# ISLA-UH/quantum-inferno

Measured on AMD Instinct MI355X. Metric: TFR Mpoints/sec (CWT+STX+entropy), higher is better.
Workload: dtype f32; 1 GPU; BASELINE configs[1]: 1 channel(s) per GPU x 2^20 samples @ 1000 Hz, order N=3, CWT+STX+entropy, 48 bands; channels_per_gpu=1, n=1048576, bands=48, engine=auto, world_size=1, backend=none, gather_message_bytes_per_rank=0

## Files before the change

### quantum_inferno_amd/csrc/qi_block.hip

```cpp
#include "qi_common.hpp"
#include "qi_device.hpp"
#include "qi_native.hpp"
#include "qi_fft_reg.hpp"
#include "qi_zoom_gather.hpp"

namespace qi {
namespace native {

namespace {

constexpr int kBlkThreads = 256;
#ifndef QI_BLK_WAVES
#define QI_BLK_WAVES 3
#endif
#ifndef QI_BLK_LONG_WAVES
#define QI_BLK_LONG_WAVES 2
#endif
#ifdef QI_NATIVE_DEBUG
#define QI_BDBG(bit) (a.debug & (bit))
#else
#define QI_BDBG(bit) false
#endif
#ifdef QI_NATIVE_STAMPS
#define QI_BSTAMP(k)                                               \
// ... 451 lines not shown
    }
    QI_BSTAMP(4);
  }
#ifdef QI_NATIVE_STAMPS
  if (a.stamps && tid == 0) {
    unsigned long long* o = a.stamps + ((int64_t)blockIdx.z * gridDim.x + blockIdx.x) * 8;
    for (int k = 0; k < 5; ++k) o[k] = st_acc[k];
    o[5] = (unsigned long long)band_count;
  }
#endif

  T tot = T(0);
  char* __restrict__ time_row = reinterpret_cast<char*>(
      a.time_part ? a.time_part + ((int64_t)ch * a.chunk_total + a.chunk_base + plane) * n : nullptr);
#pragma unroll
  for (int i = 0; i < NOUT; i += 2) {
    tot += col_p[i] + col_p[i + 1];
    const uint32_t tt = tb_pair + 256u * (uint32_t)i;
    if (time_row && tt < (uint32_t)n) store_real_pair(time_row, tt, col_p[i], col_p[i + 1]);
  }
  const double r0 = wave_max((double)mx), r1 = wave_sum((double)tot), r2 = wave_sum(plogp);
  __syncthreads();
  if (pending >= 0 && tid == 0) {
    double r = 0.0;
    for (int q = 0; q < NW; ++q) r += s_red[par ^ 1][q];
    a.part_band[((int64_t)ch * a.panel_bands + pending) * a.nblk + blk] = r;
  }
  if (a.part_stat) {
    double* fin = reinterpret_cast<double*>(buf);
    if (lane == 0) {
      fin[wv] = r0;
      fin[NW + wv] = r1;
// ... 732 lines not shown
  cplx<T> w;
  {
    float s, c;
    sincospif((float)col * (2.0f / 4096.0f), &s, &c);
    w = mk<T>((T)c, (T)s);
  }
  fft4096<T, 1>(v, buf, tw256, w, tid, col);
#pragma unroll
  for (int c = 0; c < 16; ++c) plane[256 * c] = v[brev(c, 4)];
}
template <typename T, bool STX, int NF>
__device__ __forceinline__ void zoom_coarse_plane_gather(const ZoomArgs<T>& a, const uint32_t plane_i,
                                                         cplx<T>* __restrict__ buf, cplx<T>* __restrict__ tw256) {
  const int tid = threadIdx.x, lane = tid & (kWave - 1);
  const int col = (tid & ~(kWave - 1)) + (lane < 32 ? 2 * lane : 2 * (lane - 32) + 1);
  const BandDesc bd = load_uniform(a.bands + *as_const(a.plane_band + plane_i));
  const uint32_t tau1 = plane_i - (uint32_t)bd.edge;
  const int64_t ch = blockIdx.z;
  const cplx<T>* __restrict__ X = a.X + ch * (a.Lf << a.x_shift);
  cplx<T> v[16];
#ifdef QI_NATIVE_DEBUG
  if (a.debug & 256) {
#pragma unroll
    for (int b = 0; b < 16; ++b) v[b] = mk<T>((T)(col + b), (T)tau1);
  } else
#endif
  zoom_gather16<T, STX, NF>(a, bd, tau1, col, X, v);
  {
    float s, c;
    sincospif((float)tid * (2.0f / 256.0f), &s, &c);
    tw256[tid] = mk<T>((T)c, (T)s);
// ... 428 lines not shown
```

### quantum_inferno_amd/csrc/qi_host.hpp

```cpp
#pragma once
#include <algorithm>
#include <cmath>
#include <cstring>
#include <map>
#include <mutex>
#include <new>
#include <tuple>
#include <vector>

#include <cstdlib>

#include "qi_common.hpp"
#include "qi_native.hpp"

namespace qi {

struct DeviceGuard {
  int prev = -1;
  bool ok = true;
  explicit DeviceGuard(int dev) {
    if (hipGetDevice(&prev) != hipSuccess) prev = -1;
    if (prev != dev) ok = hipSetDevice(dev) == hipSuccess;
  }
  ~DeviceGuard() {
// ... 183 lines not shown
  Profiler prof;
  struct NativeGroup {
    int32_t first = 0, count = 0;
    int32_t gen_first = 0, ngen = 0;
  };
  struct NativeTable {
    bool ready = false;
    int64_t Lf = 0;
    int32_t nbands = 0, ngen = 0, imd_slots = 0;
    native::BandDesc* d_bands = nullptr;
    int32_t* d_gen_list = nullptr;
    std::vector<NativeGroup> groups;
    void* Hc = nullptr;
    void* Hfull = nullptr;
    native::BandDesc* d_zoom = nullptr;
    int32_t* d_zoom_plane_band = nullptr;
    std::vector<std::pair<int32_t, int32_t>> h_zoom;
    std::vector<int32_t> h_rows;
    int32_t nzoom = 0, zoom_count[native::kZoomClasses] = {0, 0, 0, 0, 0, 0, 0};
    int64_t zoom_planes = 0;
    int zoom_max_level = 0;
    native::BandDesc* d_z64 = nullptr;
    int32_t nz64 = 0, z64_first[native::kZ64Levels] = {}, z64_count[native::kZ64Levels] = {};
    int32_t zf_first[native::kZ64FineClasses] = {}, zf_count[native::kZ64FineClasses] = {};
    double2* d_z64_lane_ph = nullptr;
    double2* d_z64_wave_ph = nullptr;
    void release() {
      if (d_z64) (void)hipFree(d_z64);
      if (d_z64_lane_ph) (void)hipFree(d_z64_lane_ph);
      if (d_z64_wave_ph) (void)hipFree(d_z64_wave_ph);
      if (d_zoom) (void)hipFree(d_zoom);
      if (d_zoom_plane_band) (void)hipFree(d_zoom_plane_band);
      if (d_bands) (void)hipFree(d_bands);
      if (d_gen_list) (void)hipFree(d_gen_list);
      if (Hc) (void)hipFree(Hc);
      if (Hfull) (void)hipFree(Hfull);
      *this = NativeTable();
    }
  } nat[4];
  struct BlockTable {
    bool ready = false;
    int demod = 0;
    void* bank = nullptr;
    int32_t rows = 0;
    struct ItemList {
      void* d_bands = nullptr;
      void* d_demod_pow = nullptr;
      void* d_gauss_w = nullptr;
      std::vector<std::pair<int32_t, int32_t>> h_bands;
      native::BlockItem* d_items = nullptr;
      int32_t nitems = 0, nplanes = 0;
      int32_t nlong = 0;
      int32_t nedge_items = 0;
      bool edge_merged = false;
      std::vector<native::BlockItem> h_items;
    } var[2];
    int64_t max_blocks = 0;
    void release() {
      if (bank) (void)hipFree(bank);
      for (auto& v : var) {
        if (v.d_bands) (void)hipFree(v.d_bands);
        if (v.d_demod_pow) (void)hipFree(v.d_demod_pow);
        if (v.d_gauss_w) (void)hipFree(v.d_gauss_w);
        if (v.d_items) (void)hipFree(v.d_items);
      }
      *this = BlockTable();
// ... 121 lines not shown
```

### quantum_inferno_amd/csrc/qi_native.hip

```cpp
#include <utility>

#include "qi_common.hpp"
#include "qi_device.hpp"
#include "qi_native.hpp"
#include "qi_fft_reg.hpp"
#include "qi_finalize.hpp"

namespace qi {
namespace native {

namespace {

template <typename T, int G_ = 16>
struct Cfg {
  static constexpr int NR = 1024, G = G_, TH = 64 * G_;
  static constexpr int SR = NR + 1;
  static constexpr int SA = 16 * G + 1;
  static constexpr int BUF = (G * SR > 64 * SA) ? G * SR : 64 * SA;
  static constexpr int TW1 = (kMaxPrunedTerms + 1) * G;
  static constexpr int TW2 = 64;
  static constexpr size_t LDS_BYTES = ((size_t)BUF + NR + TW2 + TW1) * sizeof(cplx<T>) + 256;
};

#ifdef QI_NATIVE_DEBUG
// ... 476 lines not shown
      double m = 0.0, s1 = 0.0, s2 = 0.0;
      for (int w = 0; w < C::TH / kWave; ++w) {
        m = s_fin[0][w] > m ? s_fin[0][w] : m;
        s1 += s_fin[1][w];
        s2 += s_fin[2][w];
      }
      double* o = a.part_stat + ((int64_t)ch * a.stat_stride + (int64_t)(a.chunk_base + blockIdx.y) * a.stat_nblk + grp) * 3;
      o[0] = m;
      o[1] = s1;
      o[2] = s2;
    }
  }
}

template <typename T, int VEC>
__device__ __forceinline__ void time_reduce_block(const T* __restrict__ part, T* __restrict__ out, int64_t n, int nchunk,
                                                  const T* __restrict__ edge_time, int64_t wmax, int64_t bx, int64_t gx,
                                                  int64_t c) {
  struct alignas(sizeof(T) * VEC) Pack {
    T v[VEC];
  };
  for (int64_t t = (bx * blockDim.x + threadIdx.x) * VEC; t < n; t += gx * blockDim.x * VEC) {
    if (t + VEC <= n) {
      Pack s = *reinterpret_cast<const Pack*>(part + (c * nchunk) * n + t);
      for (int q = 1; q < nchunk; ++q) {
        const Pack x = *reinterpret_cast<const Pack*>(part + (c * nchunk + q) * n + t);
#pragma unroll
        for (int i = 0; i < VEC; ++i) s.v[i] += x.v[i];
      }
      if (edge_time) {
#pragma unroll
        for (int i = 0; i < VEC; ++i) {
          if (t + i < wmax) s.v[i] += edge_time[(c * 2 + 0) * wmax + t + i];
          if (t + i >= n - wmax) s.v[i] += edge_time[(c * 2 + 1) * wmax + (n - 1 - t - i)];
        }
      }
      *reinterpret_cast<Pack*>(out + c * n + t) = s;
    } else {
      for (int64_t u = t; u < n; ++u) {
        T s = T(0);
        for (int q = 0; q < nchunk; ++q) s += part[(c * nchunk + q) * n + u];
        if (edge_time) {
          if (u < wmax) s += edge_time[(c * 2 + 0) * wmax + u];
          if (u >= n - wmax) s += edge_time[(c * 2 + 1) * wmax + (n - 1 - u)];
        }
        out[c * n + u] = s;
      }
    }
  }
}
template <typename T, int VEC>
__global__ void __launch_bounds__(256) k_time_reduce(const T* __restrict__ part, T* __restrict__ out, int64_t n, int nchunk,
                                                     const T* __restrict__ edge_time, int64_t wmax) {
  time_reduce_block<T, VEC>(part, out, n, nchunk, edge_time, wmax, blockIdx.x, gridDim.x, blockIdx.y);
}

struct TailFin {
  const double* part_band;
  const double* part_stat;
  double* power_band;
  double* stats;
  int64_t B, nblk, nstat;
  const int32_t* band_slots;
};
template <typename T, int VEC>
__global__ void __launch_bounds__(256) k_tail(const T* __restrict__ part, T* __restrict__ out, int64_t n, int nchunk,
                                              const T* __restrict__ edge_time, int64_t wmax, TailFin f, int nfin) {
  __shared__ double s[3][256 / kWave];
  if ((int)blockIdx.x < nfin) {
    finalize_block(f.part_band, f.part_stat, f.power_band, f.stats, f.B, f.nblk, f.nstat, f.band_slots, blockIdx.x,
                   blockIdx.y, s);
    return;
  }
  time_reduce_block<T, VEC>(part, out, n, nchunk, edge_time, wmax, (int64_t)blockIdx.x - nfin, (int64_t)gridDim.x - nfin,
                            blockIdx.y);
}

template <typename T>
__global__ void k_even_bins(const cplx<T>* __restrict__ x2, cplx<T>* __restrict__ x1, int64_t n) {
  const int64_t k = (int64_t)blockIdx.x * blockDim.x + threadIdx.x, c = blockIdx.y;
  if (k < n) x1[c * n + k] = x2[c * 2 * n + 2 * k];
}

template <typename T>
__global__ void __launch_bounds__(256) k_edge_fix(EdgeArgs<T> a) {
  const int lane = threadIdx.x & (kWave - 1), wv = threadIdx.x / kWave;
  const int64_t e = blockIdx.y, c = blockIdx.z;
  const EdgeBand eb = a.bands[e];
  const int64_t o = (int64_t)blockIdx.x * (256 / kWave) + wv;
// ... 300 lines not shown
    return QI_ERR_UNSUPPORTED;
  }
  return launch_pass2_cfg<double, Cfg<double, 8>>(a, kind, nchunk, n_channels, st);
}

template <>
int launch_pass2<float>(const RowArgs<float>& a, int kind, int rows_per_group, int nchunk, int64_t n_channels,
                        hipStream_t st) {
  if (rows_per_group == 16) return launch_pass2_cfg<float, Cfg<float, 16>>(a, kind, nchunk, n_channels, st);
  if (rows_per_group == 8) return launch_pass2_cfg<float, Cfg<float, 8>>(a, kind, nchunk, n_channels, st);
  set_error("pass 2 supports 8 or 16 rows per workgroup, got %d", rows_per_group);
  return QI_ERR_UNSUPPORTED;
}

template <typename T>
int launch_time_reduce(const T* part, T* out, int64_t C, int64_t n, int nchunk, const T* edge_time, int64_t wmax,
                       hipStream_t st) {
  const bool aligned = n % 4 == 0 && reinterpret_cast<uintptr_t>(out) % (4 * sizeof(T)) == 0 &&
                       reinterpret_cast<uintptr_t>(part) % (4 * sizeof(T)) == 0;
  if (aligned) {
    dim3 g((unsigned)(ceil_div(n, 1024) > 4096 ? 4096 : ceil_div(n, 1024)), (unsigned)C);
    k_time_reduce<T, 4><<<g, 256, 0, st>>>(part, out, n, nchunk, edge_time, wmax);
  } else {
    dim3 g((unsigned)(ceil_div(n, 256) > 4096 ? 4096 : ceil_div(n, 256)), (unsigned)C);
    k_time_reduce<T, 1><<<g, 256, 0, st>>>(part, out, n, nchunk, edge_time, wmax);
  }
  QI_LAUNCH_CHECK();
  return QI_OK;
}
template <typename T>
struct TailPack {
  const T* part;
  T* out;
  int64_t n;
  int nchunk, nfin;
  TailFin f;
};
template <typename T, int VEC>
__global__ void __launch_bounds__(256) k_tail2(TailPack<T> p0, TailPack<T> p1) {
  __shared__ double s[3][256 / kWave];
  const TailPack<T>& p = blockIdx.z == 0 ? p0 : p1;
  if ((int)blockIdx.x < p.nfin) {
    finalize_block(p.f.part_band, p.f.part_stat, p.f.power_band, p.f.stats, p.f.B, p.f.nblk, p.f.nstat, p.f.band_slots,
                   blockIdx.x, blockIdx.y, s);
    return;
  }
  time_reduce_block<T, VEC>(p.part, p.out, p.n, p.nchunk, nullptr, 0, (int64_t)blockIdx.x - p.nfin,
                            (int64_t)gridDim.x - p.nfin, blockIdx.y);
}

template <typename T>
int launch_tail(const TailCall<T>& t, hipStream_t st) {
  const bool aligned = t.n % 4 == 0 && reinterpret_cast<uintptr_t>(t.out_time) % (4 * sizeof(T)) == 0 &&
                       reinterpret_cast<uintptr_t>(t.time_part) % (4 * sizeof(T)) == 0;
  if (!aligned) {
    if (int rc = launch_time_reduce<T>(t.time_part, t.out_time, t.ct, t.n, t.chunk_total, t.edge_time, t.wmax, st)) return rc;
    return launch_finalize(t.part_band, t.part_stat, t.power_band, t.stats, t.ct, t.B, t.nbk, t.stat_slots, st, t.band_slots);
  }
  const TailFin f{t.part_band, t.part_stat, t.power_band, t.stats, t.B, t.nbk, t.stat_slots, t.band_slots};
  const int nfin = (int)t.B + 1;
  const int64_t gt = ceil_div(t.n, 1024) > 4096 ? 4096 : ceil_div(t.n, 1024);
  dim3 g((unsigned)(gt + nfin), (unsigned)t.ct);
  k_tail<T, 4><<<g, 256, 0, st>>>(t.time_part, t.out_time, t.n, t.chunk_total, t.edge_time, t.wmax, f, nfin);
  QI_LAUNCH_CHECK();
  return QI_OK;
}

template <typename T>
int launch_tail2(const TailCall<T>& t0, const TailCall<T>& t1, hipStream_t st) {
  const int64_t n = t1.n;
  const bool aligned = n % 4 == 0 && reinterpret_cast<uintptr_t>(t0.out_time) % 16 == 0 &&
                       reinterpret_cast<uintptr_t>(t0.time_part) % 16 == 0 && reinterpret_cast<uintptr_t>(t1.out_time) % 16 == 0 &&
                       reinterpret_cast<uintptr_t>(t1.time_part) % 16 == 0;
  if (!aligned) {
    if (int rc = launch_tail<T>(t0, st)) return rc;
    return launch_tail<T>(t1, st);
  }
  TailPack<T> p0{t0.time_part, t0.out_time, n, t0.chunk_total, (int)t0.B + 1,
                 TailFin{t0.part_band, t0.part_stat, t0.power_band, t0.stats, t0.B, t0.nbk, t0.stat_slots, t0.band_slots}};
  TailPack<T> p1{t1.time_part, t1.out_time, n, t1.chunk_total, (int)t1.B + 1,
                 TailFin{t1.part_band, t1.part_stat, t1.power_band, t1.stats, t1.B, t1.nbk, t1.stat_slots, t1.band_slots}};
  const int64_t gt = ceil_div(n, 1024) > 4096 ? 4096 : ceil_div(n, 1024);
  const int nfin = p0.nfin > p1.nfin ? p0.nfin : p1.nfin;
  dim3 g((unsigned)(gt + nfin), (unsigned)t1.ct, 2);
  k_tail2<T, 4><<<g, 256, 0, st>>>(p0, p1);
  QI_LAUNCH_CHECK();
  return QI_OK;
}
template int launch_tail2<float>(const TailCall<float>&, const TailCall<float>&, hipStream_t);
template int launch_tail<float>(const TailCall<float>&, hipStream_t);
template int launch_tail<double>(const TailCall<double>&, hipStream_t);
template int launch_time_reduce<float>(const float*, float*, int64_t, int64_t, int, const float*, int64_t, hipStream_t);
template int launch_time_reduce<double>(const double*, double*, int64_t, int64_t, int, const double*, int64_t,
                                        hipStream_t);

template <typename T>
int launch_even_bins(const cplx<T>* x2, cplx<T>* x1, int64_t C, int64_t n, hipStream_t st) {
  dim3 g((unsigned)ceil_div(n, 256), (unsigned)C);
  k_even_bins<T><<<g, 256, 0, st>>>(x2, x1, n);
  QI_LAUNCH_CHECK();
  return QI_OK;
}
template int launch_even_bins<float>(const float2*, float2*, int64_t, int64_t, hipStream_t);
template int launch_even_bins<double>(const double2*, double2*, int64_t, int64_t, hipStream_t);

template <typename T>
int launch_edge(const EdgeArgs<T>& a, int64_t C, T* edge_time, double* part_band, int64_t nblk, int64_t band_slot,
                double* part_stat, int64_t stat_slot, hipStream_t st) {
// ... 35 lines not shown
```

### quantum_inferno_amd/csrc/qi_native.hpp

```cpp
#pragma once
#include "qi_common.hpp"

namespace qi {
namespace native {

constexpr int kN2 = 1024;
constexpr int kMaxPrunedTerms = 16;

struct BandDesc {
  int32_t mode;
  int32_t k_lo;
  int32_t k_len;
  int32_t gen_slot;
  int32_t out_band;
  int32_t bank_row;
  int32_t edge;
  int32_t edge_slot;
  int32_t add_row;
  int32_t pad_;
  int64_t src_off;
  int64_t shift;
  double coef;
};

// ... 103 lines not shown
  const BlockItem* items;
  const BlockBandT<T>* bands;
  const cplx<T>* bank;
  const T* gauss_w;
  const cplx<T>* demod_pow;
  const cplx<T>* demod_t1;
  const cplx<T>* demod_t2;
  const T* sig;
  cplx<T>* coef;
  T* bits;
  T* time_part;
  double* part_band;
  double* part_stat;
  int64_t nblk, stat_stride, stat_base;
  int32_t chunk_base, chunk_total;
  T power_scale, eps;
  float two_over_n;
  int32_t debug;
  unsigned long long* stamps;
};
int block_valid(int wq);
template <typename T>
int launch_block(const BlockArgs<T>& a, int demod, int64_t n_channels, hipStream_t st, hipStream_t side = nullptr,
                 hipEvent_t fork = nullptr, hipEvent_t join = nullptr);
template <typename T>
int launch_block_dual(const BlockArgs<T>& a0, const BlockArgs<T>& a2, const DualItem* items, int32_t nitems, int32_t nlong,
                      int32_t n_edge, int64_t n_channels, hipStream_t st);
int launch_block_taps_gabor(double2* g, int w, const double* d_par, int nb_total, const int32_t* d_ids, int count,
                            hipStream_t st);
int launch_block_taps_stx(double2* g, int w, const double2* om, int64_t n, int64_t idx, hipStream_t st);
// ... 7 lines not shown
constexpr int kZoomLevels = 5;
constexpr int kZoomClasses = 7;
constexpr int zoom_grid(int cls) { return cls < kZoomLevels ? cls : 0; }
constexpr int zoom_ntap(int cls) { return cls < kZoomLevels ? 10 : (cls == 5 ? 6 : 4); }
constexpr int zoom_design_oversampling(int cls) { return cls < kZoomLevels ? 4 : (cls == 5 ? 8 : 32); }
constexpr int zoom_span(int cls) { return 1 << zoom_grid(cls); }
constexpr int zoom_taps(int cls) { return zoom_ntap(cls) + zoom_span(cls) - 1; }
constexpr int zoom_steps(int cls) { return zoom_grid(cls) <= 2 ? 16 : (64 >> zoom_grid(cls)); }
constexpr int kZoomOversample = 4;
template <typename T>
struct ZoomArgs {
  int64_t n, Lf;
  int64_t planes;
  int32_t nbands, panel_bands;
  const BandDesc* bands;
  const int32_t* plane_band;
  int32_t lvl_first[kZoomClasses], lvl_count[kZoomClasses], lvl_chunk0[kZoomClasses], lvl_nchunk[kZoomClasses];
  int64_t lvl_stat_base[kZoomClasses];
  const float* lvl_weights[kZoomClasses];
  const cplx<T>* X;
  int32_t x_shift;
  const cplx<T>* Hc;
  cplx<T>* split_part;
  int32_t split_rows;
  int32_t debug;
  cplx<T>* coarse;
  int32_t stx;
  int32_t lane_off;
  int64_t tau_off;
  T inv_len;
  float two_over_len;
// ... 73 lines not shown
  int32_t cls;
  int32_t nrow;
  int32_t lvl_bands;
  int32_t lvl_index0;
  const double* w;
  const cplx<double>* lane_ph;
  const cplx<double>* wave_ph;
  int32_t debug;
};
int launch_z64_fine(const Z64FineArgs& a, int64_t n_channels, hipStream_t st);
void z64_fine_weights(int cls, double* w );

void zoom_weights(int level, int lane_off, float* w );

template <typename T>
int launch_time_reduce(const T* part, T* out, int64_t C, int64_t n, int nchunk, const T* edge_time, int64_t wmax,
                       hipStream_t st);
template <typename T>
struct TailCall {
  const T* time_part = nullptr;
  T* out_time = nullptr;
  int64_t ct = 0, n = 0;
  int chunk_total = 0;
  const T* edge_time = nullptr;
  int64_t wmax = 0;
  const double* part_band = nullptr;
  const double* part_stat = nullptr;
  double* power_band = nullptr;
  double* stats = nullptr;
  int64_t B = 0, nbk = 0, stat_slots = 0;
  const int32_t* band_slots = nullptr;
};
template <typename T>
int launch_tail(const TailCall<T>& t, hipStream_t st);
template <typename T>
int launch_tail2(const TailCall<T>& t0, const TailCall<T>& t1, hipStream_t st);
template <typename T>
int launch_even_bins(const cplx<T>* x2, cplx<T>* x1, int64_t C, int64_t n, hipStream_t st);
// ... 11 lines not shown
```

### quantum_inferno_amd/csrc/qi_plan_build.hip

```cpp
#include <algorithm>

#include "qi_host.hpp"

using namespace qi;

namespace qi {
namespace host {

bool native_len_ok(int64_t Lf) { return Lf == (1ll << 20) || Lf == (1ll << 21); }

bool native_wanted(const qi_plan* p, int kind) {
  if (p->d.engine == QI_ENGINE_HIPFFT) return false;
  const int64_t Lf = kind == 0 ? p->L : p->n;
  if (p->d.dtype == QI_F64 && !p->native_f64) return false;
  if (is_pow2(p->n) && native_len_ok(Lf)) return true;
  return kind != 1 && is_pow2(p->n) && p->n >= ((int64_t)1 << p->native_min_log2n) && Lf <= (1ll << 26);
}

bool z64_table(const qi_plan* p, int table) { return p->d.dtype == QI_F64 && p->native_z64 && table != 3; }
int64_t narrow_limit(const qi_plan* p, int table, int64_t Lf) {
  return z64_table(p, table) ? std::max<int64_t>(p->native_kmax, Lf >> (9 - p->native_z64_levels)) : p->native_kmax;
}

int batch_from(const qi_plan* p) {
// ... 38 lines not shown
      const int g = kZoomListOrder[gi];
      const int grid = native::zoom_grid(g);
      for (auto d : by_level[g]) {
        d.edge_slot = grid;
        d.edge = (int32_t)t.zoom_planes;
        t.zoom_planes += ((Lf / native::kZoomD) << grid) / native::kBlk;
        if (grid > t.zoom_max_level) t.zoom_max_level = grid;
        zoom.push_back(d);
        t.h_zoom.push_back({d.out_band, g});
      }
    }
    if (!zoom.empty()) {
      QI_HIP(hipMalloc((void**)&t.d_zoom, zoom.size() * sizeof(native::BandDesc)));
      QI_HIP(hipMemcpy(t.d_zoom, zoom.data(), zoom.size() * sizeof(native::BandDesc), hipMemcpyHostToDevice));
      t.nzoom = (int32_t)zoom.size();
      std::vector<int32_t> owner((size_t)t.zoom_planes);
      for (size_t j = 0; j < zoom.size(); ++j) {
        const int64_t planes = ((Lf / native::kZoomD) << zoom[j].edge_slot) / native::kBlk;
        for (int64_t q = 0; q < planes; ++q) owner[(size_t)(zoom[j].edge + q)] = (int32_t)j;
      }
      QI_HIP(hipMalloc((void**)&t.d_zoom_plane_band, owner.size() * sizeof(int32_t)));
      QI_HIP(hipMemcpy(t.d_zoom_plane_band, owner.data(), owner.size() * sizeof(int32_t), hipMemcpyHostToDevice));
      for (int g = 0; g < native::kZoomClasses; ++g)
        for (int e = 0; e < 1; ++e) {
          const bool needed = t.zoom_count[g] > 0 || (g == 0 && t.zoom_count[5] + t.zoom_count[6] > 0);
          if (p->d_zoom_w[g][e] || !needed) continue;
          std::vector<float> w((size_t)64 * native::zoom_taps(g));
          native::zoom_weights(g, e, w.data());
          QI_HIP(hipMalloc((void**)&p->d_zoom_w[g][e], w.size() * sizeof(float)));
          QI_HIP(hipMemcpy(p->d_zoom_w[g][e], w.data(), w.size() * sizeof(float), hipMemcpyHostToDevice));
        }
    }
    bands.swap(rest);
  }
  if (z64_table(p, kind)) {
    std::vector<native::BandDesc> rest;
    std::vector<std::vector<native::BandDesc>> lvl(native::kZ64Levels);
// ... 333 lines not shown
        {
          const int64_t m1 = picks[r].shift % p->n;
          b.rot1[0] = (T)std::cos(-2.0 * M_PI * (double)m1 / (double)p->n);
          b.rot1[1] = (T)std::sin(-2.0 * M_PI * (double)m1 / (double)p->n);
        }
        list.push_back(b);
      }
      group_first[g] = first;
      group_count[g] = (int32_t)list.size() - first;
      if (group_count[g] == 0) continue;
      const int64_t nblocks = ceil_div(p->n, native::block_valid(wqs[g]));
      if (nblocks > bt.max_blocks) bt.max_blocks = nblocks;
      for (int32_t q = first; q < (int32_t)list.size(); ++q) il.h_bands.push_back({list[q].out_band, (int32_t)nblocks});
    }
    std::vector<native::BlockItem> items;
    for (int g = 0; g < NG; ++g) {
      const int32_t first = group_first[g], count = group_count[g];
      if (count == 0) continue;
      const int per_wg = v == 0 ? p->native_blk_bands : p->native_blk_bands_batch;
      const int32_t nchunk = (int32_t)ceil_div(count, per_wg);
      const int64_t nblocks = ceil_div(p->n, native::block_valid(wqs[g]));
      if (tune_env("QI_NATIVE_VERBOSE"))
        fprintf(stderr, "[qi plan] block table %d cut %d, reach <= %d%s: %d bands (%d analytic, %d narrow, %d half) in %d workgroups x %lld blocks\n", kind, v,
                g == 3 ? 1024 : 256 * (wqs[g] & 15), g == 3 ? " (8192-sample blocks)" : "", count,
                (int)std::count_if(list.begin() + first, list.begin() + first + count, [](const native::BlockBandT<T>& b) { return b.analytic != 0; }),
                (int)std::count_if(list.begin() + first, list.begin() + first + count, [](const native::BlockBandT<T>& b) { return b.narrow == 1; }),
                (int)std::count_if(list.begin() + first, list.begin() + first + count, [](const native::BlockBandT<T>& b) { return b.narrow == 2; }),
                nchunk, (long long)nblocks);
      for (int32_t c = 0; c < nchunk; ++c) {
        const int32_t lo = first + (int32_t)((int64_t)count * c / nchunk);
        const int32_t hi = first + (int32_t)((int64_t)count * (c + 1) / nchunk);
        for (int64_t b = 0; b < nblocks; ++b) {
          native::BlockItem it;
          it.wq = wqs[g];
          it.block = (int32_t)b;
          it.band_first = lo;
          it.band_count = hi - lo;
          it.plane = il.nplanes;
          it.stat_slot = 0;
          items.push_back(it);
        }
        il.nplanes += 1;
      }
    }
    std::stable_sort(items.begin(), items.end(), [](const native::BlockItem& x, const native::BlockItem& y) {
      const bool lx = x.wq == native::kBlkLongWq, ly = y.wq == native::kBlkLongWq;
      return lx != ly ? lx : x.band_count > y.band_count;
    });
    for (size_t i = 0; i < items.size(); ++i) items[i].stat_slot = (int32_t)i;
    il.nitems = (int32_t)items.size();
    il.nlong = (int32_t)std::count_if(items.begin(), items.end(), [](const native::BlockItem& x) { return x.wq == native::kBlkLongWq; });
    if (kind == 0 && p->nsplit > 0) {
      const int wq = (int)(p->native_split_e / 512);
      il.edge_merged = (v == 1 && p->native_edge_merge != 0) || F64;
      if (il.edge_merged) {
// ... 484 lines not shown
```

### quantum_inferno_amd/csrc/qi_run.hip

```cpp
#include "qi_host.hpp"

using namespace qi;

namespace qi {
namespace host {



struct Tile {
  int64_t Ct, Bt, ntb, nblk;
  size_t off_x, off_y, off_pb, off_ps;
};

template <typename T>
int plan_tiles(const qi_plan* p, int64_t C, int64_t B, int64_t L, Tile* t) {
  const size_t row = (size_t)L * sizeof(cplx<T>);
  const int64_t nblk = ceil_div(p->n, kEpiSpan);
  const size_t part = align_up((size_t)B * nblk * 8) + align_up((size_t)B * nblk * 24);
  const size_t per_chan_full = row * (size_t)(B + 1) + part + 2048;
  int64_t Ct, Bt;
  if (per_chan_full <= p->ws_bytes) {
    Bt = B;
    Ct = (int64_t)(p->ws_bytes / per_chan_full);
    if (Ct > C) Ct = C;
// ... 533 lines not shown
  v.fill_panel(e);
  e.edge_z = s.edge_z;
  e.edge_p = s.edge_p;
  return native::launch_edge<T>(e, ct, v.out_time ? s.edge_time : nullptr, v.part_band, v.nbk, v.nbk - 1, v.part_stat,
                                v.stat_slots - p->nedge, st);
}

template <typename T>
native::TailCall<T> tail_call(const TileOut<T>& v, int64_t ct, const int32_t* band_slots) {
  native::TailCall<T> t;
  t.time_part = v.time_part;
  t.out_time = v.out_time;
  t.ct = ct;
  t.n = v.n;
  t.chunk_total = v.chunk_total;
  t.part_band = v.part_band;
  t.part_stat = v.part_stat;
  t.power_band = v.power_band;
  t.stats = v.stats;
  t.B = v.B;
  t.nbk = v.nbk;
  t.stat_slots = v.stat_slots;
  t.band_slots = band_slots;
  return t;
}

template <typename T>
int launch_reductions(const native::TailCall<T>& t, bool time_via_part, bool one_launch, hipStream_t st) {
  const bool sums = t.part_band || t.part_stat;
  if (time_via_part && sums && one_launch) return native::launch_tail<T>(t, st);
  if (time_via_part)
    QI_TRY(native::launch_time_reduce<T>(t.time_part, t.out_time, t.ct, t.n, t.chunk_total, t.edge_time, t.wmax, st));
  if (sums)
    QI_TRY(launch_finalize(t.part_band, t.part_stat, t.power_band, t.stats, t.ct, t.B, t.nbk, t.stat_slots, st, t.band_slots));
  return QI_OK;
}


struct ZoomRows {
  int count[native::kZoomClasses] = {}, nchunk[native::kZoomClasses] = {};
  int64_t stat_base[native::kZoomClasses] = {}, groups[native::kZoomClasses] = {};
  int planes = 0;
  int64_t stats = 0, slots = 0;
};

ZoomRows plan_zoom_rows(const qi_plan* p, int kind, int64_t C, bool joint) {
  constexpr int NL = native::kZoomClasses;
// ... 70 lines not shown
  return QI_OK;
}

native::ZoomArgs<float> zoom_args(const qi_plan* p, int kind, const ZoomRows& r, const TileOut<float>& v, const Scratch<float>& s,
                                  bool x_shift, int32_t nsplit, int64_t stat_base, int chunk_base) {
  using T = float;
  const auto& zt = p->nat[kind];
  const int64_t n = v.n;
  native::ZoomArgs<T> z{};
  z.n = n;
  z.Lf = zt.Lf;
  z.planes = zt.zoom_planes;
  z.nbands = zt.nzoom;
  z.panel_bands = (int32_t)v.B;
  z.bands = zt.d_zoom;
  z.plane_band = zt.d_zoom_plane_band;
  z.X = s.X;
  z.x_shift = x_shift ? 1 : 0;
  z.Hc = static_cast<const cplx<T>*>(zt.Hc);
  z.coarse = s.zoom;
  z.stx = kind == 2 ? 1 : 0;
  z.lane_off = kind == 0 ? 1 : 0;
  z.tau_off = kind == 2 ? 0 : n / 2 / native::kZoomD;
  z.inv_len = (T)(1.0 / (double)zt.Lf);
  z.two_over_len = (float)(2.0 / (double)zt.Lf);
  v.fill(z);
  z.chunk_base = chunk_base;
  z.split_part = s.zadd;
  z.split_rows = nsplit;
  z.debug = p->native_debug;
  int chunk0 = 0;
// ... 108 lines not shown
    blk_stats = il.nitems + il.nedge_items;
    blk_slots = bt.max_blocks;
  }
  const auto& zt = p->nat[kind];
  const bool zoom = zt.nzoom > 0;
  const ZoomRows zr = plan_zoom_rows(p, kind, C, defer || (finish && (finish->active || probe)));
  const int chunk_z0 = chunk_total;
  chunk_total += zr.planes;
  int64_t nbk = tp.nblk_max + (shorts ? 1 : 0);
  if (blk_slots > nbk) nbk = blk_slots;
  if (zr.slots > nbk) nbk = zr.slots;
  const int64_t p2_stats = (int64_t)chunk_p2 * tp.nblk_max;
  const int64_t stat_slots = p2_stats + blk_stats + zr.stats + (shorts ? p->nedge : 0);
  const bool sums = out->power_band || out->stats;
  const bool time_via_part = out->power_time && (chunk_total > 1 || shorts);
  if (!shorts) QI_TRY(upload_band_slots(p, kind, cut, tp.nblk_max, blocks));
  const int32_t* band_slots = shorts ? nullptr : p->d_band_slots[kind][cut];
  bool share = may_share && kind == 2 && (probe || (p->shared_valid && p->shared_sig == sig_v && p->shared_C == C)) &&
               p->nat[kind].h_rows.empty() && !shorts;
  const int32_t nsplit = kind == 0 ? p->nsplit : 0;
  ScratchBytes e = scratch_bytes<T>(p, n, B, nbk, stat_slots, chunk_total, shorts, time_via_part, out->coef != nullptr, nsplit);
  e.x = (size_t)(share ? 2 * Lf0 : Lf0) * sizeof(cplx<T>);
  e.imd = (size_t)(tp.imd_elems < Lf0 ? Lf0 : tp.imd_elems) * sizeof(cplx<T>);
  e.zoom = zoom ? (size_t)zt.zoom_planes * native::kBlk * sizeof(cplx<T>) : 0;
  const size_t per_chan = e.per_record();
  if (probe) {
    *probe = per_chan;
    return QI_OK;
  }
  if (p->ws_bytes < per_chan + 4096) {
// ... 38 lines not shown
    const TileOut<T> v = tile_out<T>(out, c0, B, n, time_via_part ? s.time_part : nullptr, s.part_band, s.part_stat, nbk,
                                     stat_slots, chunk_total);
    if (shorts) QI_HIP(hipMemsetAsync(s.parts0, 0, s.parts_bytes, st));
    QI_TRY(launch_spectra<T>(p, sig_t, n, Lf0, shorts, share, s, ct, st));
    QI_TRY(launch_two_pass<T>(p, tp, v, s, G, tp.nblk_max, true, ct, st));
    if (zoom)
      QI_TRY(launch_zoom_stage(p, zoom_args(p, kind, zr, v, s, share, nsplit, p2_stats + blk_stats, chunk_z0), zt.zoom_max_level,
                               deferring && p->native_fuse > 2 ? defer : nullptr, finishing ? finish : nullptr, ct, st));
    if (finishing && finish->has_zoom) {
      QI_TRY(launch_zoom_all(p, finish->zoom, finish->ct, st));
      finish->has_zoom = false;
    }
    if (blocks) {
      native::BlockArgs<T> b = block_args<T>(p, bt, il, v, sig_t, s.zadd, nsplit, p2_stats, chunk_p2);
      b.nlong = il.nlong;
      QI_TRY(launch_block_stage(p, b, bt.demod, cut, deferring ? defer : nullptr, finishing ? finish : nullptr, ct, st));
    }
    p->prof.begin(st, QI_STAGE_EPILOGUE);
    if (shorts) QI_TRY(launch_edges<T>(p, v, s, sig_t, ct, st));
    native::TailCall<T> tc = tail_call<T>(v, ct, band_slots);
    if (deferring) {
      defer->tail = tc;
      defer->ws_used = (size_t)(ar.w - p->ws);
      defer->active = true;
    } else if (finishing) {
      QI_TRY(launch_tails(finish, tc, st));
    } else {
      tc.edge_time = shorts ? s.edge_time : nullptr;
      tc.wmax = p->edge_wmax;
      QI_TRY(launch_reductions<T>(tc, time_via_part, p->native_tail != 0, st));
    }
    p->prof.end(QI_STAGE_EPILOGUE, st);
  }
  return QI_OK;
}
// ... 210 lines not shown
```

### quantum_inferno_amd/csrc/qi_zoom.hip

```cpp
#include "qi_common.hpp"
#include "qi_device.hpp"
#include "qi_native.hpp"
#include "qi_fft_reg.hpp"
#include "qi_zoom_gather.hpp"

namespace qi {
namespace native {

namespace {

constexpr int kZoomThreads = 256;

__device__ __forceinline__ float lane_value(float v, int lane) {
  return __uint_as_float(__builtin_amdgcn_readlane(__float_as_uint(v), lane));
}

template <typename T, bool STX>
__device__ __forceinline__ void zoom_gather_plane(const ZoomArgs<T>& a, const uint32_t plane) {
  const BandDesc bd = load_uniform(a.bands + *as_const(a.plane_band + plane));
  const int32_t kappa0 = (int32_t)(blockIdx.x * 256 + threadIdx.x);
  const uint32_t tau1 = plane - (uint32_t)bd.edge;
  const int64_t ch = blockIdx.z;
  const cplx<T>* __restrict__ X = a.X + ch * (a.Lf << a.x_shift);
  a.coarse[((int64_t)ch * a.planes + bd.edge) * kBlk + (int32_t)tau1 * kBlk + kappa0] =
      zoom_gather_value<T, STX>(a, bd, tau1, kappa0, X);
}
template <typename T, bool STX>
__global__ void __launch_bounds__(256) k_zoom_gather(ZoomArgs<T> a) {
  zoom_gather_plane<T, STX>(a, blockIdx.y);
}
template <typename T>
__global__ void __launch_bounds__(256) k_zoom_gather2(ZoomArgs<T> a0, ZoomArgs<T> a2) {
  if (blockIdx.y < (uint32_t)a0.planes) zoom_gather_plane<T, false>(a0, blockIdx.y);
  else zoom_gather_plane<T, true>(a2, blockIdx.y - (uint32_t)a0.planes);
// ... 334 lines not shown
```

Before: 407,900 Mpoints/s.

## Fold zoom time partials into one block plane and store band descriptors per plane

Picks one non-long block plane at plan-build time to act as collector. That block plane sums the zoom-stage time partial rows into its own column before storing them. The tail time reduction then sums only the chunks before the zoom range, cutting how many partial rows the final reduce reads. Zoom kernels also now read a per-plane BandDesc directly instead of chasing a plane-to-band index, which removes one dependent load at the cost of a larger table. The collector plane gains extra serial global reads, which could lengthen that block and create imbalance.

```diff
diff --git a/quantum_inferno_amd/csrc/qi_block.hip b/quantum_inferno_amd/csrc/qi_block.hip
--- a/quantum_inferno_amd/csrc/qi_block.hip
+++ b/quantum_inferno_amd/csrc/qi_block.hip
@@ -489,8 +489,43 @@
   char* __restrict__ time_row = reinterpret_cast<char*>(
       a.time_part ? a.time_part + ((int64_t)ch * a.chunk_total + a.chunk_base + plane) * n : nullptr);
 #pragma unroll
+  for (int i = 0; i < NOUT; i += 2) tot += col_p[i] + col_p[i + 1];
+  if constexpr (!EDGE && !F64) {
+    if (time_row && a.collect_count > 0 && plane == a.collect_plane) {
+      T zs[NOUT];
+#pragma unroll
+      for (int i = 0; i < NOUT; ++i) zs[i] = T(0);
+      const char* __restrict__ zrow =
+          reinterpret_cast<const char*>(a.time_part + ((int64_t)ch * a.chunk_total + a.collect_first) * n);
+      constexpr int G = 2;
+      for (int q = 0; q < a.collect_count; q += G, zrow += G * (size_t)n * sizeof(T)) {
+        float2 x[G][NOUT / 2];
+#pragma unroll
+        for (int u = 0; u < G; ++u) {
+          const bool on = q + u < a.collect_count;
+          const char* __restrict__ r = zrow + (size_t)u * (size_t)n * sizeof(T);
+#pragma unroll
+          for (int i = 0; i < NOUT; i += 2) {
+            const uint32_t tt = tb_pair + 256u * (uint32_t)i;
+            x[u][i / 2] = on && tt < (uint32_t)n ? *reinterpret_cast<const float2*>(r + (size_t)(tt * (uint32_t)sizeof(T)))
+                                                 : make_float2(0.0f, 0.0f);
+          }
+        }
+#pragma unroll
+        for (int u = 0; u < G; ++u) {
+#pragma unroll
+          for (int i = 0; i < NOUT; i += 2) {
+            zs[i] += x[u][i / 2].x;
+            zs[i + 1] += x[u][i / 2].y;
+          }
+        }
+      }
+#pragma unroll
+      for (int i = 0; i < NOUT; ++i) col_p[i] = zs[i] + col_p[i];
+    }
+  }
+#pragma unroll
   for (int i = 0; i < NOUT; i += 2) {
-    tot += col_p[i] + col_p[i + 1];
     const uint32_t tt = tb_pair + 256u * (uint32_t)i;
     if (time_row && tt < (uint32_t)n) store_real_pair(time_row, tt, col_p[i], col_p[i + 1]);
   }
@@ -1253,7 +1288,7 @@
                                                          cplx<T>* __restrict__ buf, cplx<T>* __restrict__ tw256) {
   const int tid = threadIdx.x, lane = tid & (kWave - 1);
   const int col = (tid & ~(kWave - 1)) + (lane < 32 ? 2 * lane : 2 * (lane - 32) + 1);
-  const BandDesc bd = load_uniform(a.bands + *as_const(a.plane_band + plane_i));
+  const BandDesc bd = load_uniform(a.plane_desc + plane_i);
   const uint32_t tau1 = plane_i - (uint32_t)bd.edge;
   const int64_t ch = blockIdx.z;
   const cplx<T>* __restrict__ X = a.X + ch * (a.Lf << a.x_shift);
diff --git a/quantum_inferno_amd/csrc/qi_host.hpp b/quantum_inferno_amd/csrc/qi_host.hpp
--- a/quantum_inferno_amd/csrc/qi_host.hpp
+++ b/quantum_inferno_amd/csrc/qi_host.hpp
@@ -221,7 +221,7 @@
     void* Hc = nullptr;
     void* Hfull = nullptr;
     native::BandDesc* d_zoom = nullptr;
-    int32_t* d_zoom_plane_band = nullptr;
+    native::BandDesc* d_zoom_plane_desc = nullptr;
     std::vector<std::pair<int32_t, int32_t>> h_zoom;
     std::vector<int32_t> h_rows;
     int32_t nzoom = 0, zoom_count[native::kZoomClasses] = {0, 0, 0, 0, 0, 0, 0};
@@ -237,7 +237,7 @@
       if (d_z64_lane_ph) (void)hipFree(d_z64_lane_ph);
       if (d_z64_wave_ph) (void)hipFree(d_z64_wave_ph);
       if (d_zoom) (void)hipFree(d_zoom);
-      if (d_zoom_plane_band) (void)hipFree(d_zoom_plane_band);
+      if (d_zoom_plane_desc) (void)hipFree(d_zoom_plane_desc);
       if (d_bands) (void)hipFree(d_bands);
       if (d_gen_list) (void)hipFree(d_gen_list);
       if (Hc) (void)hipFree(Hc);
@@ -257,6 +257,7 @@
       std::vector<std::pair<int32_t, int32_t>> h_bands;
       native::BlockItem* d_items = nullptr;
       int32_t nitems = 0, nplanes = 0;
+      int32_t collect_plane = -1;
       int32_t nlong = 0;
       int32_t nedge_items = 0;
       bool edge_merged = false;
diff --git a/quantum_inferno_amd/csrc/qi_native.hip b/quantum_inferno_amd/csrc/qi_native.hip
--- a/quantum_inferno_amd/csrc/qi_native.hip
+++ b/quantum_inferno_amd/csrc/qi_native.hip
@@ -514,7 +514,7 @@
 }
 
 template <typename T, int VEC>
-__device__ __forceinline__ void time_reduce_block(const T* __restrict__ part, T* __restrict__ out, int64_t n, int nchunk,
+__device__ __forceinline__ void time_reduce_block(const T* __restrict__ part, T* __restrict__ out, int64_t n, int nchunk, int nsum,
                                                   const T* __restrict__ edge_time, int64_t wmax, int64_t bx, int64_t gx,
                                                   int64_t c) {
   struct alignas(sizeof(T) * VEC) Pack {
@@ -523,7 +523,7 @@
   for (int64_t t = (bx * blockDim.x + threadIdx.x) * VEC; t < n; t += gx * blockDim.x * VEC) {
     if (t + VEC <= n) {
       Pack s = *reinterpret_cast<const Pack*>(part + (c * nchunk) * n + t);
-      for (int q = 1; q < nchunk; ++q) {
+      for (int q = 1; q < nsum; ++q) {
         const Pack x = *reinterpret_cast<const Pack*>(part + (c * nchunk + q) * n + t);
 #pragma unroll
         for (int i = 0; i < VEC; ++i) s.v[i] += x.v[i];
@@ -539,7 +539,7 @@
     } else {
       for (int64_t u = t; u < n; ++u) {
         T s = T(0);
-        for (int q = 0; q < nchunk; ++q) s += part[(c * nchunk + q) * n + u];
+        for (int q = 0; q < nsum; ++q) s += part[(c * nchunk + q) * n + u];
         if (edge_time) {
           if (u < wmax) s += edge_time[(c * 2 + 0) * wmax + u];
           if (u >= n - wmax) s += edge_time[(c * 2 + 1) * wmax + (n - 1 - u)];
@@ -551,8 +551,8 @@
 }
 template <typename T, int VEC>
 __global__ void __launch_bounds__(256) k_time_reduce(const T* __restrict__ part, T* __restrict__ out, int64_t n, int nchunk,
-                                                     const T* __restrict__ edge_time, int64_t wmax) {
-  time_reduce_block<T, VEC>(part, out, n, nchunk, edge_time, wmax, blockIdx.x, gridDim.x, blockIdx.y);
+                                                     int nsum, const T* __restrict__ edge_time, int64_t wmax) {
+  time_reduce_block<T, VEC>(part, out, n, nchunk, nsum, edge_time, wmax, blockIdx.x, gridDim.x, blockIdx.y);
 }
 
 struct TailFin {
@@ -564,7 +564,7 @@
   const int32_t* band_slots;
 };
 template <typename T, int VEC>
-__global__ void __launch_bounds__(256) k_tail(const T* __restrict__ part, T* __restrict__ out, int64_t n, int nchunk,
+__global__ void __launch_bounds__(256) k_tail(const T* __restrict__ part, T* __restrict__ out, int64_t n, int nchunk, int nsum,
                                               const T* __restrict__ edge_time, int64_t wmax, TailFin f, int nfin) {
   __shared__ double s[3][256 / kWave];
   if ((int)blockIdx.x < nfin) {
@@ -572,7 +572,7 @@
                    blockIdx.y, s);
     return;
   }
-  time_reduce_block<T, VEC>(part, out, n, nchunk, edge_time, wmax, (int64_t)blockIdx.x - nfin, (int64_t)gridDim.x - nfin,
+  time_reduce_block<T, VEC>(part, out, n, nchunk, nsum, edge_time, wmax, (int64_t)blockIdx.x - nfin, (int64_t)gridDim.x - nfin,
                             blockIdx.y);
 }
 
@@ -903,16 +903,16 @@
 }
 
 template <typename T>
-int launch_time_reduce(const T* part, T* out, int64_t C, int64_t n, int nchunk, const T* edge_time, int64_t wmax,
+int launch_time_reduce(const T* part, T* out, int64_t C, int64_t n, int nchunk, int nsum, const T* edge_time, int64_t wmax,
                        hipStream_t st) {
   const bool aligned = n % 4 == 0 && reinterpret_cast<uintptr_t>(out) % (4 * sizeof(T)) == 0 &&
                        reinterpret_cast<uintptr_t>(part) % (4 * sizeof(T)) == 0;
   if (aligned) {
     dim3 g((unsigned)(ceil_div(n, 1024) > 4096 ? 4096 : ceil_div(n, 1024)), (unsigned)C);
-    k_time_reduce<T, 4><<<g, 256, 0, st>>>(part, out, n, nchunk, edge_time, wmax);
+    k_time_reduce<T, 4><<<g, 256, 0, st>>>(part, out, n, nchunk, nsum, edge_time, wmax);
   } else {
     dim3 g((unsigned)(ceil_div(n, 256) > 4096 ? 4096 : ceil_div(n, 256)), (unsigned)C);
-    k_time_reduce<T, 1><<<g, 256, 0, st>>>(part, out, n, nchunk, edge_time, wmax);
+    k_time_reduce<T, 1><<<g, 256, 0, st>>>(part, out, n, nchunk, nsum, edge_time, wmax);
   }
   QI_LAUNCH_CHECK();
   return QI_OK;
@@ -922,7 +922,7 @@
   const T* part;
   T* out;
   int64_t n;
-  int nchunk, nfin;
+  int nchunk, nsum, nfin;
   TailFin f;
 };
 template <typename T, int VEC>
@@ -934,7 +934,7 @@
                    blockIdx.x, blockIdx.y, s);
     return;
   }
-  time_reduce_block<T, VEC>(p.part, p.out, p.n, p.nchunk, nullptr, 0, (int64_t)blockIdx.x - p.nfin,
+  time_reduce_block<T, VEC>(p.part, p.out, p.n, p.nchunk, p.nsum, nullptr, 0, (int64_t)blockIdx.x - p.nfin,
                             (int64_t)gridDim.x - p.nfin, blockIdx.y);
 }
 
@@ -943,14 +943,14 @@
   const bool aligned = t.n % 4 == 0 && reinterpret_cast<uintptr_t>(t.out_time) % (4 * sizeof(T)) == 0 &&
                        reinterpret_cast<uintptr_t>(t.time_part) % (4 * sizeof(T)) == 0;
   if (!aligned) {
-    if (int rc = launch_time_reduce<T>(t.time_part, t.out_time, t.ct, t.n, t.chunk_total, t.edge_time, t.wmax, st)) return rc;
+    if (int rc = launch_time_reduce<T>(t.time_part, t.out_time, t.ct, t.n, t.chunk_total, t.chunk_sum, t.edge_time, t.wmax, st)) return rc;
     return launch_finalize(t.part_band, t.part_stat, t.power_band, t.stats, t.ct, t.B, t.nbk, t.stat_slots, st, t.band_slots);
   }
   const TailFin f{t.part_band, t.part_stat, t.power_band, t.stats, t.B, t.nbk, t.stat_slots, t.band_slots};
   const int nfin = (int)t.B + 1;
   const int64_t gt = ceil_div(t.n, 1024) > 4096 ? 4096 : ceil_div(t.n, 1024);
   dim3 g((unsigned)(gt + nfin), (unsigned)t.ct);
-  k_tail<T, 4><<<g, 256, 0, st>>>(t.time_part, t.out_time, t.n, t.chunk_total, t.edge_time, t.wmax, f, nfin);
+  k_tail<T, 4><<<g, 256, 0, st>>>(t.time_part, t.out_time, t.n, t.chunk_total, t.chunk_sum, t.edge_time, t.wmax, f, nfin);
   QI_LAUNCH_CHECK();
   return QI_OK;
 }
@@ -965,9 +965,9 @@
     if (int rc = launch_tail<T>(t0, st)) return rc;
     return launch_tail<T>(t1, st);
   }
-  TailPack<T> p0{t0.time_part, t0.out_time, n, t0.chunk_total, (int)t0.B + 1,
+  TailPack<T> p0{t0.time_part, t0.out_time, n, t0.chunk_total, t0.chunk_sum, (int)t0.B + 1,
                  TailFin{t0.part_band, t0.part_stat, t0.power_band, t0.stats, t0.B, t0.nbk, t0.stat_slots, t0.band_slots}};
-  TailPack<T> p1{t1.time_part, t1.out_time, n, t1.chunk_total, (int)t1.B + 1,
+  TailPack<T> p1{t1.time_part, t1.out_time, n, t1.chunk_total, t1.chunk_sum, (int)t1.B + 1,
                  TailFin{t1.part_band, t1.part_stat, t1.power_band, t1.stats, t1.B, t1.nbk, t1.stat_slots, t1.band_slots}};
   const int64_t gt = ceil_div(n, 1024) > 4096 ? 4096 : ceil_div(n, 1024);
   const int nfin = p0.nfin > p1.nfin ? p0.nfin : p1.nfin;
@@ -979,8 +979,8 @@
 template int launch_tail2<float>(const TailCall<float>&, const TailCall<float>&, hipStream_t);
 template int launch_tail<float>(const TailCall<float>&, hipStream_t);
 template int launch_tail<double>(const TailCall<double>&, hipStream_t);
-template int launch_time_reduce<float>(const float*, float*, int64_t, int64_t, int, const float*, int64_t, hipStream_t);
-template int launch_time_reduce<double>(const double*, double*, int64_t, int64_t, int, const double*, int64_t,
+template int launch_time_reduce<float>(const float*, float*, int64_t, int64_t, int, int, const float*, int64_t, hipStream_t);
+template int launch_time_reduce<double>(const double*, double*, int64_t, int64_t, int, int, const double*, int64_t,
                                         hipStream_t);
 
 template <typename T>
diff --git a/quantum_inferno_amd/csrc/qi_native.hpp b/quantum_inferno_amd/csrc/qi_native.hpp
--- a/quantum_inferno_amd/csrc/qi_native.hpp
+++ b/quantum_inferno_amd/csrc/qi_native.hpp
@@ -141,6 +141,7 @@
   double* part_stat;
   int64_t nblk, stat_stride, stat_base;
   int32_t chunk_base, chunk_total;
+  int32_t collect_plane, collect_first, collect_count;
   T power_scale, eps;
   float two_over_n;
   int32_t debug;
@@ -178,7 +179,7 @@
   int64_t planes;
   int32_t nbands, panel_bands;
   const BandDesc* bands;
-  const int32_t* plane_band;
+  const BandDesc* plane_desc;
   int32_t lvl_first[kZoomClasses], lvl_count[kZoomClasses], lvl_chunk0[kZoomClasses], lvl_nchunk[kZoomClasses];
   int64_t lvl_stat_base[kZoomClasses];
   const float* lvl_weights[kZoomClasses];
@@ -282,7 +283,7 @@
 void zoom_weights(int level, int lane_off, float* w );
 
 template <typename T>
-int launch_time_reduce(const T* part, T* out, int64_t C, int64_t n, int nchunk, const T* edge_time, int64_t wmax,
+int launch_time_reduce(const T* part, T* out, int64_t C, int64_t n, int nchunk, int nsum, const T* edge_time, int64_t wmax,
                        hipStream_t st);
 template <typename T>
 struct TailCall {
@@ -290,6 +291,7 @@
   T* out_time = nullptr;
   int64_t ct = 0, n = 0;
   int chunk_total = 0;
+  int chunk_sum = 0;
   const T* edge_time = nullptr;
   int64_t wmax = 0;
   const double* part_band = nullptr;
diff --git a/quantum_inferno_amd/csrc/qi_plan_build.hip b/quantum_inferno_amd/csrc/qi_plan_build.hip
--- a/quantum_inferno_amd/csrc/qi_plan_build.hip
+++ b/quantum_inferno_amd/csrc/qi_plan_build.hip
@@ -76,13 +76,13 @@
       QI_HIP(hipMalloc((void**)&t.d_zoom, zoom.size() * sizeof(native::BandDesc)));
       QI_HIP(hipMemcpy(t.d_zoom, zoom.data(), zoom.size() * sizeof(native::BandDesc), hipMemcpyHostToDevice));
       t.nzoom = (int32_t)zoom.size();
-      std::vector<int32_t> owner((size_t)t.zoom_planes);
+      std::vector<native::BandDesc> owner((size_t)t.zoom_planes);
       for (size_t j = 0; j < zoom.size(); ++j) {
         const int64_t planes = ((Lf / native::kZoomD) << zoom[j].edge_slot) / native::kBlk;
-        for (int64_t q = 0; q < planes; ++q) owner[(size_t)(zoom[j].edge + q)] = (int32_t)j;
-      }
-      QI_HIP(hipMalloc((void**)&t.d_zoom_plane_band, owner.size() * sizeof(int32_t)));
-      QI_HIP(hipMemcpy(t.d_zoom_plane_band, owner.data(), owner.size() * sizeof(int32_t), hipMemcpyHostToDevice));
+        for (int64_t q = 0; q < planes; ++q) owner[(size_t)(zoom[j].edge + q)] = zoom[j];
+      }
+      QI_HIP(hipMalloc((void**)&t.d_zoom_plane_desc, owner.size() * sizeof(native::BandDesc)));
+      QI_HIP(hipMemcpy(t.d_zoom_plane_desc, owner.data(), owner.size() * sizeof(native::BandDesc), hipMemcpyHostToDevice));
       for (int g = 0; g < native::kZoomClasses; ++g)
         for (int e = 0; e < 1; ++e) {
           const bool needed = t.zoom_count[g] > 0 || (g == 0 && t.zoom_count[5] + t.zoom_count[6] > 0);
@@ -446,6 +446,7 @@
       for (int32_t q = first; q < (int32_t)list.size(); ++q) il.h_bands.push_back({list[q].out_band, (int32_t)nblocks});
     }
     std::vector<native::BlockItem> items;
+    int32_t collect_bands = 0;
     for (int g = 0; g < NG; ++g) {
       const int32_t first = group_first[g], count = group_count[g];
       if (count == 0) continue;
@@ -471,6 +472,10 @@
           it.plane = il.nplanes;
           it.stat_slot = 0;
           items.push_back(it);
+        }
+        if (!F64 && wqs[g] != native::kBlkLongWq && hi - lo > collect_bands) {
+          collect_bands = hi - lo;
+          il.collect_plane = il.nplanes;
         }
         il.nplanes += 1;
       }
diff --git a/quantum_inferno_amd/csrc/qi_run.hip b/quantum_inferno_amd/csrc/qi_run.hip
--- a/quantum_inferno_amd/csrc/qi_run.hip
+++ b/quantum_inferno_amd/csrc/qi_run.hip
@@ -571,6 +571,7 @@
   t.ct = ct;
   t.n = v.n;
   t.chunk_total = v.chunk_total;
+  t.chunk_sum = v.chunk_total;
   t.part_band = v.part_band;
   t.part_stat = v.part_stat;
   t.power_band = v.power_band;
@@ -587,7 +588,7 @@
   const bool sums = t.part_band || t.part_stat;
   if (time_via_part && sums && one_launch) return native::launch_tail<T>(t, st);
   if (time_via_part)
-    QI_TRY(native::launch_time_reduce<T>(t.time_part, t.out_time, t.ct, t.n, t.chunk_total, t.edge_time, t.wmax, st));
+    QI_TRY(native::launch_time_reduce<T>(t.time_part, t.out_time, t.ct, t.n, t.chunk_total, t.chunk_sum, t.edge_time, t.wmax, st));
   if (sums)
     QI_TRY(launch_finalize(t.part_band, t.part_stat, t.power_band, t.stats, t.ct, t.B, t.nbk, t.stat_slots, st, t.band_slots));
   return QI_OK;
@@ -688,7 +689,7 @@
   z.nbands = zt.nzoom;
   z.panel_bands = (int32_t)v.B;
   z.bands = zt.d_zoom;
-  z.plane_band = zt.d_zoom_plane_band;
+  z.plane_desc = zt.d_zoom_plane_desc;
   z.X = s.X;
   z.x_shift = x_shift ? 1 : 0;
   z.Hc = static_cast<const cplx<T>*>(zt.Hc);
@@ -827,6 +828,7 @@
   const int64_t stat_slots = p2_stats + blk_stats + zr.stats + (shorts ? p->nedge : 0);
   const bool sums = out->power_band || out->stats;
   const bool time_via_part = out->power_time && (chunk_total > 1 || shorts);
+  const bool collect = time_via_part && zoom && blocks && il.collect_plane >= 0;
   if (!shorts) QI_TRY(upload_band_slots(p, kind, cut, tp.nblk_max, blocks));
   const int32_t* band_slots = shorts ? nullptr : p->d_band_slots[kind][cut];
   bool share = may_share && kind == 2 && (probe || (p->shared_valid && p->shared_sig == sig_v && p->shared_C == C)) &&
@@ -895,11 +897,17 @@
     if (blocks) {
       native::BlockArgs<T> b = block_args<T>(p, bt, il, v, sig_t, s.zadd, nsplit, p2_stats, chunk_p2);
       b.nlong = il.nlong;
+      if (collect) {
+        b.collect_plane = il.collect_plane;
+        b.collect_first = chunk_z0;
+        b.collect_count = zr.planes;
+      }
       QI_TRY(launch_block_stage(p, b, bt.demod, cut, deferring ? defer : nullptr, finishing ? finish : nullptr, ct, st));
     }
     p->prof.begin(st, QI_STAGE_EPILOGUE);
     if (shorts) QI_TRY(launch_edges<T>(p, v, s, sig_t, ct, st));
     native::TailCall<T> tc = tail_call<T>(v, ct, band_slots);
+    if (collect) tc.chunk_sum = chunk_z0;
     if (deferring) {
       defer->tail = tc;
       defer->ws_used = (size_t)(ar.w - p->ws);
diff --git a/quantum_inferno_amd/csrc/qi_zoom.hip b/quantum_inferno_amd/csrc/qi_zoom.hip
--- a/quantum_inferno_amd/csrc/qi_zoom.hip
+++ b/quantum_inferno_amd/csrc/qi_zoom.hip
@@ -17,7 +17,7 @@
 
 template <typename T, bool STX>
 __device__ __forceinline__ void zoom_gather_plane(const ZoomArgs<T>& a, const uint32_t plane) {
-  const BandDesc bd = load_uniform(a.bands + *as_const(a.plane_band + plane));
+  const BandDesc bd = load_uniform(a.plane_desc + plane);
   const int32_t kappa0 = (int32_t)(blockIdx.x * 256 + threadIdx.x);
   const uint32_t tau1 = plane - (uint32_t)bd.edge;
   const int64_t ch = blockIdx.z;
```

New measurement: 412,500 Mpoints/s, median of 6. +1.1%, better.
